# GuidoManni/BodySLAM

Measured on AMD Instinct MI355X. Metric: frames/sec depth+pose+back-proj, 640x480 seq, higher is better.
Workload: dtype f16

## Files before the change

bodyslam_amd/csrc/igemm_kernel.h:

```cpp
#pragma once
#include <type_traits>

#include "common.h"

namespace bs {

struct IgemmParams {
    const void* A;
    const void* W;
    const void* zero;
    long long a_bytes;
    int M, N, K, lda;
    int Hin, Win, Cin, Hout, Wout, KH, KW, stride, pad_h, pad_w;
    int tiles_per_tap;
    int cin1;
    int split_off;
    int res_split_off;
    int relu_a;
    const float* bias;
    int bias_group_rows;
    int act;
    const float* scale;
    const void* res;
    const void* res2;
    int res_dtype, ldr;
    void* out;
    void* out2;
    void* out3;
    int out_dtype, ldo, out_mode;
    int out_group_rows, out_group_stride, out_row_offset;
    int shuffle_s, shuffle_cout;
    int qkv_hidden, qkv_tokens, qkv_sp;
    int qkv_cls_last;
    int qkv_cls_rows;
    int qkv_patch_row0;
    int qkv_lo_off;
    int f8_wonly_from;
    float q_scale;
    int ntm, ntn;
    int m_begin;
    int f8_seg;
    int f8_sa0, f8_sb0, f8_sa1, f8_sb1;
    int f8_stages;
    int res_f8;
    int out_f8;
    int out2_relu;
    int out_lo8_rows;
    int f8_skip_from;
    int out_planes_rows;
    const float* bias2;
    int bias2_row0, bias2_group_rows;
    int strip;
    int ablate;
};

template <typename T>
__device__ __forceinline__ typename T16<T>::v8 relu8(typename T16<T>::v8 x) {
    typedef short s16x8 __attribute__((ext_vector_type(8)));
    s16x8 b = __builtin_bit_cast(s16x8, x);
    s16x8 neg = b >> 15;
    b = b & ~neg;
    return __builtin_bit_cast(typename T16<T>::v8, b);
}

template <typename T>
__device__ __forceinline__ void store4(void* base, int64_t off, int out_dtype, const float (&y)[4], int split_off = 0) {
    if (split_off > 0) {
        typename T16<T>::v4 h, l;
#pragma unroll
        for (int e = 0; e < 4; ++e) {
            h[e] = T16<T>::from_f32(y[e]);
            l[e] = T16<T>::from_f32(y[e] - T16<T>::to_f32(h[e]));
        }
        *reinterpret_cast<typename T16<T>::v4*>(reinterpret_cast<T*>(base) + off) = h;
        *reinterpret_cast<typename T16<T>::v4*>(reinterpret_cast<T*>(base) + off + split_off) = l;
        return;
    }
    if (out_dtype == BS_F32) {
        f32x4 v = {y[0], y[1], y[2], y[3]};
        *reinterpret_cast<f32x4*>(reinterpret_cast<float*>(base) + off) = v;
    } else {
        typename T16<T>::v4 v;
        v[0] = T16<T>::from_f32(y[0]);
        v[1] = T16<T>::from_f32(y[1]);
        v[2] = T16<T>::from_f32(y[2]);
        v[3] = T16<T>::from_f32(y[3]);
        *reinterpret_cast<typename T16<T>::v4*>(reinterpret_cast<T*>(base) + off) = v;
    }
}

template <typename T>
__device__ __forceinline__ void store8(void* base, int64_t off, int out_dtype, const float (&y)[8], int split_off = 0) {
    typedef typename T16<T>::v8 v8;
    if (split_off > 0) {
        v8 h, l;
#pragma unroll
        for (int e = 0; e < 8; ++e) {
            h[e] = T16<T>::from_f32(y[e]);
            l[e] = T16<T>::from_f32(y[e] - T16<T>::to_f32(h[e]));
        }
        *reinterpret_cast<v8*>(reinterpret_cast<T*>(base) + off) = h;
        *reinterpret_cast<v8*>(reinterpret_cast<T*>(base) + off + split_off) = l;
        return;
    }
    if (out_dtype == BS_F32) {
        *reinterpret_cast<f32x4*>(reinterpret_cast<float*>(base) + off) = f32x4{y[0], y[1], y[2], y[3]};
        *reinterpret_cast<f32x4*>(reinterpret_cast<float*>(base) + off + 4) = f32x4{y[4], y[5], y[6], y[7]};
    } else {
        v8 v;
#pragma unroll
        for (int e = 0; e < 8; ++e) v[e] = T16<T>::from_f32(y[e]);
        *reinterpret_cast<v8*>(reinterpret_cast<T*>(base) + off) = v;
    }
}

template <typename T>
__device__ __forceinline__ void store8_f8(void* base, int64_t row_off, int n, int plane_off, const float (&y)[8], int ea, int el, bool lo = true,
                                          bool hi8 = true) {
    typedef typename T16<T>::v8 v8;
    typedef int i32x2 __attribute__((ext_vector_type(2)));
    v8 h;
    f32x2_ yh[4];
    const float sa = __builtin_ldexpf(1.0f, ea), sl = __builtin_ldexpf(1.0f, el);
    const f32x2_ sa2 = {sa, sa}, sl2 = {sl, sl};
#pragma unroll
    for (int e = 0; e < 8; e += 2) {
        h[e] = T16<T>::from_f32(y[e]);
        h[e + 1] = T16<T>::from_f32(y[e + 1]);
        const f32x2_ v = f32x2_{y[e], y[e + 1]} * sa2;
        yh[e >> 1] = f32x2_{__builtin_amdgcn_fmed3f(v[0], -448.0f, 448.0f), __builtin_amdgcn_fmed3f(v[1], -448.0f, 448.0f)};
    }
    T* rowp = reinterpret_cast<T*>(base) + row_off;
    *reinterpret_cast<v8*>(rowp + n) = h;
    if (!hi8) return;
    int ph0 = 0, ph1 = 0;
    ph0 = __builtin_amdgcn_cvt_pk_fp8_f32(yh[0][0], yh[0][1], ph0, false);
    ph0 = __builtin_amdgcn_cvt_pk_fp8_f32(yh[1][0], yh[1][1], ph0, true);
    ph1 = __builtin_amdgcn_cvt_pk_fp8_f32(yh[2][0], yh[2][1], ph1, false);
    ph1 = __builtin_amdgcn_cvt_pk_fp8_f32(yh[3][0], yh[3][1], ph1, true);
    char* bytes = reinterpret_cast<char*>(rowp + plane_off);
    *reinterpret_cast<i32x2*>(bytes + n) = i32x2{ph0, ph1};
    if (lo) {
        f32x2_ yl[4];
#pragma unroll
        for (int e = 0; e < 8; e += 2) {
            const f32x2_ r = (f32x2_{y[e], y[e + 1]} + f32x2_{-T16<T>::to_f32(h[e]), -T16<T>::to_f32(h[e + 1])}) * sl2;
            yl[e >> 1] = f32x2_{__builtin_amdgcn_fmed3f(r[0], -448.0f, 448.0f), __builtin_amdgcn_fmed3f(r[1], -448.0f, 448.0f)};
        }
        int pl0 = 0, pl1 = 0;
        pl0 = __builtin_amdgcn_cvt_pk_fp8_f32(yl[0][0], yl[0][1], pl0, false);
        pl0 = __builtin_amdgcn_cvt_pk_fp8_f32(yl[1][0], yl[1][1], pl0, true);
        pl1 = __builtin_amdgcn_cvt_pk_fp8_f32(yl[2][0], yl[2][1], pl1, false);
        pl1 = __builtin_amdgcn_cvt_pk_fp8_f32(yl[3][0], yl[3][1], pl1, true);
        *reinterpret_cast<i32x2*>(bytes + plane_off + n) = i32x2{pl0, pl1};
    }
}

template <typename T>
__device__ __forceinline__ void add_lo8(float* y, const void* base, int64_t row_off, int C, int n) {
    const char* lp = reinterpret_cast<const char*>(reinterpret_cast<const T*>(base) + row_off + C + (C >> 1)) + n;
    const int packed = *reinterpret_cast<const int*>(lp);
    typedef float f32x2 __attribute__((ext_vector_type(2)));
    const f32x2 a = __builtin_amdgcn_cvt_pk_f32_fp8(packed, false), b = __builtin_amdgcn_cvt_pk_f32_fp8(packed, true);
    const float sc = __builtin_ldexpf(1.0f, -BS_F8_ACT_LO_EXP);
    y[0] += a[0] * sc; y[1] += a[1] * sc; y[2] += b[0] * sc; y[3] += b[1] * sc;
}

constexpr int NW_CHECK(int a, int b) { return a * b; }

template <int N>
__device__ __forceinline__ void wait_vmcnt() {
    asm volatile("s_waitcnt vmcnt(%0)" ::"n"(N) : "memory");
}

template <typename T, int BM, int BN, int WM, int WN, int BK, int STAGES, int MODE, bool PP = false, int CM = 0, int SCHED = 0>
__global__ __launch_bounds__(WM* WN * 64, 2) void igemm_kernel(const IgemmParams p) {
#if defined(__HIP_DEVICE_COMPILE__)
    constexpr bool CONV = MODE != 0;
    constexpr bool RELU_A = MODE == 2;
    constexpr bool F8 = CM != 0;
    constexpr int NT = WM * WN * 64;
    constexpr int ROWB = BK * 2;
    constexpr int LPR = ROWB / 16;
    constexpr int RPR = NT / LPR;
    constexpr int RPW = 64 / LPR;
    constexpr int RA = BM / RPR, RB = BN / RPR;
    static_assert(BK == 64 || BK == 32, "BK");
    static_assert(BM % RPR == 0 && BN % RPR == 0, "tile rows must be a multiple of the DMA round");
    constexpr int GL = RA + RB;
    static_assert(GL * (STAGES - 1) <= 63, "vmcnt range");
    constexpr int TM = BM / WM, TN = BN / WN;
    constexpr int FM = TM / 16, FN = TN / 16;
    static_assert(TM % 16 == 0 && TN % 16 == 0, "wave tile must be a multiple of 16");
    constexpr int A_BYTES = BM * ROWB, B_BYTES = BN * ROWB, STAGE = A_BYTES + B_BYTES;
    constexpr int LDS_BYTES = STAGES * STAGE;
    constexpr unsigned OOB = 0x80000000u;
    typedef typename T16<T>::v8 v8;

    extern __shared__ __attribute__((aligned(16))) char smem[];

    const int nwg = gridDim.x, bid = blockIdx.x;
    const int xq = nwg >> 3, xr = nwg & 7, xcd = bid & 7, loc = bid >> 3;
    const int wg = (xcd < xr ? xcd * (xq + 1) : xr * (xq + 1) + (xcd - xr) * xq) + loc;
    int tm, tn;
    if (p.strip > 0) {
        const int per = p.ntm * p.strip, s = wg / per, r = wg - s * per;
        const int wl = p.ntn - s * p.strip < p.strip ? p.ntn - s * p.strip : p.strip;
        tm = r / wl;
        tn = s * p.strip + (r - tm * wl);
    } else {
        tm = wg / p.ntn;
        tn = wg - tm * p.ntn;
    }

    const int tid = threadIdx.x, lane = tid & 63;
    const int wave = __builtin_amdgcn_readfirstlane(tid >> 6);
    const int wm = wave / WN, wn = wave - wm * WN;
    const int srow = tid / LPR;
    const int sswz = (BK == 64) ? (srow & 7) : ((0 - (srow >> 2)) & 3);
    const int cs16 = ((tid & (LPR - 1)) ^ sswz) * 16;

    const int m0 = p.m_begin + tm * BM;
    long long a_base_el;
    int img0 = 0;
    if (CONV) {
        img0 = m0 / (p.Hout * p.Wout);
        a_base_el = (long long)img0 * p.Hin * p.Win * p.lda;
    } else {
        a_base_el = (long long)m0 * p.lda;
    }
    long long a_left = p.a_bytes - a_base_el * 2;
    a_left = a_left > 0x7FFFFFF0ll ? 0x7FFFFFF0ll : a_left;
    const __amdgpu_buffer_rsrc_t a_rsrc = __builtin_amdgcn_make_buffer_rsrc(
        const_cast<T*>(reinterpret_cast<const T*>(p.A)) + a_base_el, 0, (int)a_left, 0x00020000);
    const int w_pitch = p.K * 2;
    const __amdgpu_buffer_rsrc_t w_rsrc = __builtin_amdgcn_make_buffer_rsrc(
        const_cast<void*>(p.W), 0, (int)((long long)p.N * w_pitch), 0x00020000);

    unsigned a_off[RA];
    unsigned a_mask[RA];
#pragma unroll
    for (int j = 0; j < RA; ++j) {
        int m = m0 + j * RPR + srow;
        m = m < p.M ? m : p.M - 1;
        if (CONV) {
            const int hw = p.Hout * p.Wout;
            const int b = m / hw, rem = m - b * hw;
            const int oy = rem / p.Wout, ox = rem - oy * p.Wout;
            const int iy0 = oy * p.stride - p.pad_h, ix0 = ox * p.stride - p.pad_w;
            a_off[j] = (unsigned)((((b - img0) * p.Hin + iy0) * p.Win + ix0) * p.lda * 2 + cs16);
            unsigned mk = 0;
            for (int ky = 0; ky < p.KH; ++ky)
                for (int kx = 0; kx < p.KW; ++kx) {
                    const bool ok = (unsigned)(iy0 + ky) < (unsigned)p.Hin && (unsigned)(ix0 + kx) < (unsigned)p.Win;
                    mk |= (ok ? 1u : 0u) << (ky * p.KW + kx);
                }
            a_mask[j] = mk;
        } else {
            a_off[j] = (unsigned)((m - m0) * p.lda * 2 + cs16);
            a_mask[j] = 1u;
        }
    }
    static_assert(BN % 32 == 0 && TN % 32 == 0, "column permutation works on 32-column groups");
    unsigned w_off[RB];
#pragma unroll
    for (int j = 0; j < RB; ++j) {
        int r = j * RPR + srow;
        if (SCHED == 1) r = (((r >> 5) & 3) << 6) | ((r >> 7) << 5) | (r & 31);
        int n = tn * BN + ((r & ~31) | ((r & 12) << 1) | ((r & 16) >> 2) | (r & 3));
        n = n < p.N ? n : p.N - 1;
        w_off[j] = (unsigned)(n * w_pitch + cs16);
    }
    const int seg0 = (CONV ? p.Cin : p.K - p.cin1) * 2, seg1 = p.cin1 * 2;
    const int ntaps = CONV ? p.KH * p.KW : 1;
    int s_tap = 0, s_kx = 0, s_tapoff = 0, s_cb = 0, s_sub = 0, s_k = 0, s_seg = seg0;

    auto stage_advance = [&]() {
        s_k += BK * 2;
        if (BK == 32) {
            s_sub ^= 64;
            if (s_sub) return;
        }
        if (CONV) {
            ++s_tap;
            s_tapoff += p.lda * 2;
            if (++s_kx >= p.KW) {
                s_kx = 0;
                s_tapoff += (p.Win - p.KW) * p.lda * 2;
            }
        }
        if (!CONV || s_tap >= ntaps) {
            s_tap = 0;
            s_kx = 0;
            s_tapoff = 0;
            s_cb += 128;
            if (s_cb >= s_seg) {
                s_cb = 0;
                s_seg = seg1;
            }
        }
    };
    auto stage = [&](int buf) {
        char* sa = smem + buf * STAGE;
        char* sb = sa + A_BYTES;
        const int s_c0 = s_cb + s_sub;
#pragma unroll
        for (int j = 0; j < RA; ++j) {
            unsigned vo;
// ... 425 lines not shown
                }
                float yall[FN / 2][8];
#pragma unroll
                for (int jp = 0; jp < FN / 2; ++jp) {
                    float (&y8)[8] = yall[jp];
#pragma unroll
                    for (int h = 0; h < 2; ++h) {
                        const int j = jp * 2 + h;
                        float* y = y8 + h * 4;
                        if (n0j[j] >= p.N) continue;
                        f32x4 bsum = brow ? *reinterpret_cast<const f32x4*>(brow + n0j[j]) : bj[j];
                        if (brow2) bsum += *reinterpret_cast<const f32x4*>(brow2 + n0j[j]);
#pragma unroll
                        for (int e = 0; e < 4; ++e) y[e] = acc[i][j][e] + bsum[e];
                        const bool res32 = p.res && p.res_dtype == BS_F32;
                        if (ACT == BS_ACT_GELU) {
                            const f32x2_ g0 = gelu_erf2(f32x2_{y[0], y[1]}), g1 = gelu_erf2(f32x2_{y[2], y[3]});
                            y[0] = g0[0]; y[1] = g0[1]; y[2] = g1[0]; y[3] = g1[1];
                        }
#pragma unroll
                        for (int e = 0; e < 4; ++e) {
                            if (ACT == BS_ACT_RELU) y[e] = fmaxf(y[e], 0.0f);
                            else if (ACT == BS_ACT_SOFTPLUS) y[e] = softplus20(y[e]);
                            else if (ACT == BS_ACT_SOFTPLUS_FAST) y[e] = softplus_fast(y[e]);
                            if (!res32) y[e] *= sj[j][e];
                        }
                        if (p.res) {
                            const int64_t ro = orow * p.ldr + n0j[j];
                            if (p.res_dtype == BS_F32) {
                                const f32x4 rr = *reinterpret_cast<const f32x4*>(reinterpret_cast<const float*>(p.res) + ro);
#pragma unroll
                                for (int e = 0; e < 4; ++e) y[e] = __builtin_fmaf(y[e], sj[j][e], rr[e]);
                            } else {
                                const typename T16<T>::v4 rr = *reinterpret_cast<const typename T16<T>::v4*>(reinterpret_cast<const T*>(p.res) + ro);
#pragma unroll
                                for (int e = 0; e < 4; ++e) y[e] += T16<T>::to_f32(rr[e]);
                                if (p.res_split_off > 0) {
                                    const typename T16<T>::v4 rl = *reinterpret_cast<const typename T16<T>::v4*>(reinterpret_cast<const T*>(p.res) + ro + p.res_split_off);
#pragma unroll
                                    for (int e = 0; e < 4; ++e) y[e] += T16<T>::to_f32(rl[e]);
                                } else if (F8 && p.res_f8) {
                                    add_lo8<T>(y, p.res, orow * p.ldr, p.N, n0j[j]);
                                }
                            }
                            if (p.res2) {
                                const typename T16<T>::v4 rr = *reinterpret_cast<const typename T16<T>::v4*>(reinterpret_cast<const T*>(p.res2) + ro);
#pragma unroll
                                for (int e = 0; e < 4; ++e) y[e] += T16<T>::to_f32(rr[e]);
                                if (p.res_split_off > 0) {
                                    const typename T16<T>::v4 rl = *reinterpret_cast<const typename T16<T>::v4*>(reinterpret_cast<const T*>(p.res2) + ro + p.res_split_off);
#pragma unroll
                                    for (int e = 0; e < 4; ++e) y[e] += T16<T>::to_f32(rl[e]);
                                } else if (F8 && p.res_f8) {
                                    add_lo8<T>(y, p.res2, orow * p.ldr, p.N, n0j[j]);
                                }
                            }
                        }
                    }
                }
#pragma unroll
                for (int jp = 0; jp < FN / 2; ++jp) {
                    float (&y8)[8] = yall[jp];
                    const int j0 = jp * 2, j1 = j0 + 1;
                    if (n0j[j0] >= p.N) continue;
                    void* dst = (p.out_mode == BS_OUT_QKV && which[j0] == 1) ? p.out2 : p.out;
                    const int so = p.out_mode != BS_OUT_QKV ? p.split_off : p.qkv_lo_off;
                    if (F8 && p.out_f8) {
                        const int nloc = p.out_mode == BS_OUT_SHUFFLE ? n0j[j0] % p.shuffle_cout : n0j[j0];
                        store8_f8<T>(dst, roff + coff[j0] - nloc, nloc, so, y8, p.out_f8 & 0xff, (p.out_f8 >> 8) & 0xff);
                    } else if (wide_ok && n0j[j1] < p.N && coff[j1] == coff[j0] + 4 && which[j1] == which[j0]) {
                        store8<T>(dst, roff + coff[j0], p.out_dtype, y8, so);
                    } else {
                        const float(&ya)[4] = *reinterpret_cast<const float(*)[4]>(y8);
                        store4<T>(dst, roff + coff[j0], p.out_dtype, ya, so);
                        if (n0j[j1] < p.N) {
                            const float(&yb)[4] = *reinterpret_cast<const float(*)[4]>(y8 + 4);
                            void* dst1 = (p.out_mode == BS_OUT_QKV && which[j1] == 1) ? p.out2 : p.out;
                            store4<T>(dst1, roff + coff[j1], p.out_dtype, yb, so);
                        }
                    }
                }
            }
        };
        const bool plain_full = p.out_mode == BS_OUT_PLAIN && !p.out_group_rows && p.bias && !p.bias_group_rows && p.N % BN == 0 &&
                                p.ldo % 8 == 0 && !b2_rows && !(p.ablate & 16);
        if (plain_full && p.act == BS_ACT_NONE && p.res && p.res_dtype == BS_F32 && !p.res2 && p.out_dtype == BS_F32 && p.split_off == 0 &&
            !(F8 && p.out_f8) && p.scale && p.ldr % 4 == 0) {
            BS_FRESH_LANE
            constexpr int NP = FM * (FN / 2), DEPTH = 8;
            const float* resp = reinterpret_cast<const float*>(p.res);
            float* outp = reinterpret_cast<float*>(p.out);
            f32x4 bj[FN], sj[FN];
#pragma unroll
            for (int j = 0; j < FN; ++j) {
                const int n0 = n_wave + (j >> 1) * 32 + fq * 8 + (j & 1) * 4;
                bj[j] = *reinterpret_cast<const f32x4*>(p.bias + n0);
                if (g2 >= 0) bj[j] += *reinterpret_cast<const f32x4*>(p.bias2 + (int64_t)g2 * p.N + n0);
                sj[j] = *reinterpret_cast<const f32x4*>(p.scale + n0);
            }
            const int mrow = m0 + wm * TM + frow;
            f32x4 rq[DEPTH][2];
            auto issue = [&](int it, int slot) {
                const int i = it / (FN / 2), jp = it - i * (FN / 2);
                int m = mrow + i * 16;
                m = m < p.M ? m : p.M - 1;
                const float* rp = resp + (int64_t)m * p.ldr + n_wave + jp * 32 + fq * 8;
                rq[slot][0] = *reinterpret_cast<const f32x4*>(rp);
                rq[slot][1] = *reinterpret_cast<const f32x4*>(rp + 4);
            };
#pragma unroll
            for (int it = 0; it < DEPTH; ++it) issue(it, it);
#pragma unroll
            for (int it = 0; it < NP; ++it) {
                const int i = it / (FN / 2), jp = it - i * (FN / 2);
                const int m = mrow + i * 16;
                f32x4 y0, y1;
#pragma unroll
                for (int e = 0; e < 4; ++e) {
                    y0[e] = __builtin_fmaf(acc[i][2 * jp][e] + bj[2 * jp][e], sj[2 * jp][e], rq[it % DEPTH][0][e]);
                    y1[e] = __builtin_fmaf(acc[i][2 * jp + 1][e] + bj[2 * jp + 1][e], sj[2 * jp + 1][e], rq[it % DEPTH][1][e]);
                }
                if (it + DEPTH < NP) issue(it + DEPTH, it % DEPTH);
                if (m < p.M) {
                    float* op = outp + (int64_t)m * p.ldo + n_wave + jp * 32 + fq * 8;
                    *reinterpret_cast<f32x4*>(op) = y0;
                    *reinterpret_cast<f32x4*>(op + 4) = y1;
                }
            }
            return;
        }
        if constexpr (F8) {
            if (p.out_mode == BS_OUT_PLAIN && !p.out_group_rows && !p.bias_group_rows && p.N % BN == 0 && p.ldo % 8 == 0 && !b2_rows &&
                !(p.ablate & (16 | 2048)) && p.out_f8 && !p.scale && (p.act == BS_ACT_NONE || p.act == BS_ACT_RELU) && p.split_off == p.N &&
                p.N % 8 == 0 && p.out_dtype != BS_F32 &&
                (!p.res || (p.res_f8 && p.res_dtype != BS_F32 && p.res_split_off == 0 && p.ldr % 8 == 0)) && (!p.res2 || p.res)) {
                BS_FRESH_LANE
                typedef typename T16<T>::v8 v8;
                typedef int i32x2 __attribute__((ext_vector_type(2)));
                typedef float f32x2 __attribute__((ext_vector_type(2)));
                constexpr int NP = FM * (FN / 2), RDEPTH = 4;
                f32x4 bj[FN];
#pragma unroll
                for (int j = 0; j < FN; ++j) {
                    const int n0 = n_wave + (j >> 1) * 32 + fq * 8 + (j & 1) * 4;
                    bj[j] = p.bias ? *reinterpret_cast<const f32x4*>(p.bias + n0) : f32x4{0.f, 0.f, 0.f, 0.f};
                    if (g2 >= 0) bj[j] += *reinterpret_cast<const f32x4*>(p.bias2 + (int64_t)g2 * p.N + n0);
                }
                const bool relu = p.act == BS_ACT_RELU;
                const int mrow = m0 + wm * TM + frow;
                const int ea = p.out_f8 & 0xff, el = (p.out_f8 >> 8) & 0xff;
                const bool lo_plane = !(p.out_lo8_rows > 0 && m0 >= p.out_lo8_rows);
                const bool hi_plane = !(p.out_planes_rows > 0 && m0 >= p.out_planes_rows);
                const float lsc = __builtin_ldexpf(1.0f, -BS_F8_ACT_LO_EXP);
                auto body = [&](auto nres_tag) {
                    constexpr int NRES = decltype(nres_tag)::value;
                    v8 rh[NRES ? RDEPTH : 1][NRES ? NRES : 1];
                    i32x2 rl[NRES ? RDEPTH : 1][NRES ? NRES : 1];
                    auto issue = [&](int it, int slot) {
                        const int i = it / (FN / 2), jp = it - i * (FN / 2);
                        int m = mrow + i * 16;
                        m = m < p.M ? m : p.M - 1;
                        const int n = n_wave + jp * 32 + fq * 8;
#pragma unroll
                        for (int q = 0; q < NRES; ++q) {
                            const T* rp = reinterpret_cast<const T*>(q ? p.res2 : p.res) + (int64_t)m * p.ldr;
                            rh[slot][q] = *reinterpret_cast<const v8*>(rp + n);
                            rl[slot][q] = *reinterpret_cast<const i32x2*>(reinterpret_cast<const char*>(rp + p.N + (p.N >> 1)) + n);
                        }
                    };
                    if constexpr (NRES > 0) {
#pragma unroll
                        for (int it = 0; it < RDEPTH; ++it) issue(it, it);
                    }
#pragma unroll
                    for (int it = 0; it < NP; ++it) {
                        const int i = it / (FN / 2), jp = it - i * (FN / 2);
                        const int m = mrow + i * 16;
                        float y8[8];
#pragma unroll
                        for (int h = 0; h < 2; ++h)
#pragma unroll
                            for (int e = 0; e < 4; ++e) {
                                float y = acc[i][2 * jp + h][e] + bj[2 * jp + h][e];
                                if (relu) y = fmaxf(y, 0.0f);
                                y8[4 * h + e] = y;
                            }
                        if constexpr (NRES > 0) {
#pragma unroll
                            for (int q = 0; q < NRES; ++q) {
                                const v8 hv = rh[it % RDEPTH][q];
                                const i32x2 lv = rl[it % RDEPTH][q];
#pragma unroll
                                for (int h = 0; h < 2; ++h) {
#pragma unroll
                                    for (int e = 0; e < 4; ++e) y8[4 * h + e] += T16<T>::to_f32(hv[4 * h + e]);
                                    const f32x2 a = __builtin_amdgcn_cvt_pk_f32_fp8(lv[h], false), b = __builtin_amdgcn_cvt_pk_f32_fp8(lv[h], true);
                                    y8[4 * h] += a[0] * lsc; y8[4 * h + 1] += a[1] * lsc; y8[4 * h + 2] += b[0] * lsc; y8[4 * h + 3] += b[1] * lsc;
                                }
                            }
                            if (it + RDEPTH < NP) issue(it + RDEPTH, it % RDEPTH);
                        }
                        if (m < p.M) store8_f8<T>(p.out, (int64_t)m * p.ldo, n_wave + jp * 32 + fq * 8, p.split_off, y8, ea, el, lo_plane && hi_plane, hi_plane);
                        if (p.out2_relu) {
#pragma unroll
                            for (int e = 0; e < 8; ++e) y8[e] = fmaxf(y8[e], 0.0f);
                            if (m < p.M) store8_f8<T>(p.out2, (int64_t)m * p.ldo, n_wave + jp * 32 + fq * 8, p.split_off, y8, ea, el);
                        }
                    }
                };
                if (p.res2) body(std::integral_constant<int, 2>{});
                else if (p.res) body(std::integral_constant<int, 1>{});
                else body(std::integral_constant<int, 0>{});
                return;
            }
            if (plain_full && p.act == BS_ACT_GELU && !p.res && p.out_f8 && !p.scale && p.split_off == p.N && p.N % 8 == 0) {
                BS_FRESH_LANE
                const bool lo = !(p.out_lo8_rows > 0 && m0 >= p.out_lo8_rows);
                const bool planes = !(p.out_planes_rows > 0 && m0 >= p.out_planes_rows);
                f32x4 bj[FN];
#pragma unroll
                for (int j = 0; j < FN; ++j) {
                    const int n0 = n_wave + (j >> 1) * 32 + fq * 8 + (j & 1) * 4;
                    bj[j] = *reinterpret_cast<const f32x4*>(p.bias + n0);
                    if (g2 >= 0) bj[j] += *reinterpret_cast<const f32x4*>(p.bias2 + (int64_t)g2 * p.N + n0);
                }
                if constexpr (TM == 128 && TN == 64 && LDS_BYTES >= WM * WN * 16384) {
                    if (!planes && m0 + BM <= p.M && !(p.ablate & 1024)) {
                        typedef unsigned u32x4_ __attribute__((ext_vector_type(4)));
                        __syncthreads();
                        char* sw = smem + wave * 16384;
                        const int s7 = frow & 7;
                        const int wb0 = frow * 128 + ((fq ^ s7) << 4), wb1 = frow * 128 + (((4 + fq) ^ s7) << 4);
                        const int rr = lane >> 3, pc = lane & 7;
                        const int rb = rr * 128 + ((pc ^ rr) << 4);
                        T* op = reinterpret_cast<T*>(p.out) + (int64_t)(m0 + wm * TM + rr) * p.ldo + n_wave + pc * 8;
                        const int64_t step = (int64_t)8 * p.ldo;
#pragma unroll
                        for (int ip = 0; ip < FM; ip += 2) {
                            char* sr = sw + ((ip >> 1) & 1) * 4096;
#pragma unroll
                            for (int ii = 0; ii < 2; ++ii) {
                                const int i = ip + ii;
#pragma unroll
                                for (int jp = 0; jp < FN / 2; ++jp) {
                                    typename T16<T>::v8 h8v;
#pragma unroll
                                    for (int h = 0; h < 2; ++h) {
                                        const f32x4 v = acc[i][2 * jp + h] + bj[2 * jp + h];
                                        const f32x2_ g0 = gelu_erf2(f32x2_{v[0], v[1]}), g1 = gelu_erf2(f32x2_{v[2], v[3]});
                                        h8v[4 * h] = T16<T>::from_f32(g0[0]); h8v[4 * h + 1] = T16<T>::from_f32(g0[1]);
                                        h8v[4 * h + 2] = T16<T>::from_f32(g1[0]); h8v[4 * h + 3] = T16<T>::from_f32(g1[1]);
                                    }
                                    *reinterpret_cast<typename T16<T>::v8*>(sr + (jp ? wb1 : wb0) + ii * 2048) = h8v;
                                }
                            }
                            __builtin_amdgcn_fence(__ATOMIC_RELEASE, "wavefront");
                            __builtin_amdgcn_wave_barrier();
#pragma unroll
                            for (int it = 0; it < 4; ++it) {
                                *reinterpret_cast<u32x4_*>(op) = *reinterpret_cast<const u32x4_*>(sr + rb + it * 1024);
                                op += step;
                            }
                        }
                        return;
                    }
                }
#pragma unroll
                for (int i = 0; i < FM; ++i) {
                    const int m = m0 + wm * TM + i * 16 + frow;
                    if (m >= p.M) continue;
#pragma unroll
                    for (int jp = 0; jp < FN / 2; ++jp) {
                        float y8[8];
#pragma unroll
                        for (int h = 0; h < 2; ++h) {
                            const f32x4 v = acc[i][2 * jp + h] + bj[2 * jp + h];
                            const f32x2_ g0 = gelu_erf2(f32x2_{v[0], v[1]}), g1 = gelu_erf2(f32x2_{v[2], v[3]});
                            y8[4 * h] = g0[0]; y8[4 * h + 1] = g0[1]; y8[4 * h + 2] = g1[0]; y8[4 * h + 3] = g1[1];
                        }
                        if (planes) {
                            store8_f8<T>(p.out, (int64_t)m * p.ldo, n_wave + jp * 32 + fq * 8, p.split_off, y8, p.out_f8 & 0xff, (p.out_f8 >> 8) & 0xff, lo);
                        } else {
                            typename T16<T>::v8 h;
#pragma unroll
                            for (int e = 0; e < 8; ++e) h[e] = T16<T>::from_f32(y8[e]);
                            *reinterpret_cast<typename T16<T>::v8*>(reinterpret_cast<T*>(p.out) + (int64_t)m * p.ldo + n_wave + jp * 32 + fq * 8) = h;
                        }
                    }
                }
                return;
            }
        }
        if (F8 && p.out_mode == BS_OUT_QKV && p.qkv_hidden % BN == 0 && p.act == BS_ACT_NONE && !p.res && p.bias && !p.bias_group_rows && !b2_rows &&
            p.out_dtype != BS_F32 && !(p.ablate & 16)) {
            BS_FRESH_LANE
            const int part = (tn * BN) / p.qkv_hidden;
            T* dst = reinterpret_cast<T*>(part == 1 ? p.out2 : p.out);
            const float qs = part == 0 ? p.q_scale : 1.0f;
            f32x4 bj[FN], sj[FN];
            int64_t coff[FN / 2];
#pragma unroll
            for (int j = 0; j < FN; ++j) {
                const int n0 = n_wave + (j >> 1) * 32 + fq * 8 + (j & 1) * 4;
                bj[j] = *reinterpret_cast<const f32x4*>(p.bias + n0);
                if (g2 >= 0) bj[j] += *reinterpret_cast<const f32x4*>(p.bias2 + (int64_t)g2 * p.N + n0);
                sj[j] = p.scale ? *reinterpret_cast<const f32x4*>(p.scale + n0) : f32x4{1.f, 1.f, 1.f, 1.f};
#pragma unroll
                for (int e = 0; e < 4; ++e) sj[j][e] *= qs;
                if (!(j & 1)) {
                    const int rem = n0 - part * p.qkv_hidden;
                    coff[j >> 1] = (int64_t)(rem >> 6) * p.qkv_sp * 64 + (rem & 63);
                }
            }
            const int nhead = p.qkv_hidden >> 6;
            const long long q_bytes = (long long)p.qkv_cls_rows * nhead * p.qkv_sp * 128;
            if (p.qkv_cls_rows > 0 && m0 >= p.qkv_patch_row0 && p.qkv_lo_off == 0 && !(p.ablate & (128 | 256)) && q_bytes < 0x7FFFFFF0ll) {
                typedef unsigned u32x4_ __attribute__((ext_vector_type(4)));
                const __amdgpu_buffer_rsrc_t orsrc = __builtin_amdgcn_make_buffer_rsrc(dst, 0, (int)q_bytes, 0x00020000);
                const int Tk = p.qkv_tokens - 1;
                int m = m0 + wm * TM + frow;
                const int mp0 = m - p.qkv_patch_row0;
                const int ob0 = mp0 / Tk;
                int otok = mp0 - ob0 * Tk;
                const unsigned img_bytes = (unsigned)(nhead * p.qkv_sp) * 128u;
                unsigned roff = (unsigned)ob0 * img_bytes + (unsigned)otok * 128u;
                if constexpr (TM == 128 && TN == 64 && LDS_BYTES >= WM * WN * 16384) {
                    if (m0 + BM <= p.M && Tk % 8 == 0 && (m0 - p.qkv_patch_row0) % 8 == 0 && !(p.ablate & 1024)) {
                        __syncthreads();
                        char* sw = smem + wave * 16384;
                        const int s7 = frow & 7;
                        const int wb0 = frow * 128 + ((fq ^ s7) << 4), wb1 = frow * 128 + (((4 + fq) ^ s7) << 4);
#pragma unroll
                        for (int i = 0; i < FM; ++i) {
#pragma unroll
                            for (int jp = 0; jp < FN / 2; ++jp) {
                                typename T16<T>::v8 v;
#pragma unroll
                                for (int e = 0; e < 4; ++e) {
                                    v[e] = T16<T>::from_f32((acc[i][2 * jp][e] + bj[2 * jp][e]) * sj[2 * jp][e]);
                                    v[4 + e] = T16<T>::from_f32((acc[i][2 * jp + 1][e] + bj[2 * jp + 1][e]) * sj[2 * jp + 1][e]);
                                }
                                *reinterpret_cast<typename T16<T>::v8*>(sw + (jp ? wb1 : wb0) + i * 2048) = v;
                            }
                        }
                        __builtin_amdgcn_fence(__ATOMIC_RELEASE, "wavefront");
                        __builtin_amdgcn_wave_barrier();
                        const int rr = lane >> 3, pc = lane & 7;
                        const int mpl = m0 + wm * TM + rr - p.qkv_patch_row0;
                        const int obl = mpl / Tk;
                        int tokl = mpl - obl * Tk;
                        const int rem0 = n_wave - part * p.qkv_hidden;
                        unsigned ro = (unsigned)obl * img_bytes + (unsigned)tokl * 128u + (unsigned)(rem0 >> 6) * (unsigned)p.qkv_sp * 128u + pc * 16u;
                        const int rb = rr * 128 + ((pc ^ rr) << 4);
#pragma unroll
                        for (int it = 0; it < 16; ++it) {
                            const u32x4_ x = *reinterpret_cast<const u32x4_*>(sw + rb + it * 1024);
                            __builtin_amdgcn_raw_buffer_store_b128(x, orsrc, ro, 0, 0);
                            tokl += 8;
                            ro += 8u * 128u;
                            if (tokl >= Tk) {
                                tokl -= Tk;
                                ro += img_bytes - (unsigned)Tk * 128u;
                            }
                        }
                        return;
                    }
// ... 231 lines not shown
```

Baseline: 489.9.

## Stage fp8 split-plane epilogue stores through LDS for coalesced row writes

Splits store8_f8 into a conversion helper and a store, then adds an LDS-staged epilogue for the 64x64 wave tile. Per-lane scattered 16-byte and 8-byte writes of the f16 high plane and the fp8 hi/lo planes are first written to swizzled shared memory, then flushed as full contiguous row segments. The same staging is applied to the residual epilogue and to a new pixel-shuffle output path. The aim is better global store coalescing, at the cost of extra LDS traffic, wave barriers and more shared-memory use per wave.

```diff
diff --git a/bodyslam_amd/csrc/igemm_kernel.h b/bodyslam_amd/csrc/igemm_kernel.h
--- a/bodyslam_amd/csrc/igemm_kernel.h
+++ b/bodyslam_amd/csrc/igemm_kernel.h
@@ -114,12 +114,9 @@
     }
 }
 
+typedef int i32x2_ __attribute__((ext_vector_type(2)));
 template <typename T>
-__device__ __forceinline__ void store8_f8(void* base, int64_t row_off, int n, int plane_off, const float (&y)[8], int ea, int el, bool lo = true,
-                                          bool hi8 = true) {
-    typedef typename T16<T>::v8 v8;
-    typedef int i32x2 __attribute__((ext_vector_type(2)));
-    v8 h;
+__device__ __forceinline__ void cvt8_f8(const float (&y)[8], int ea, int el, bool lo, bool hi8, typename T16<T>::v8& h, i32x2_& ph, i32x2_& pl) {
     f32x2_ yh[4];
     const float sa = __builtin_ldexpf(1.0f, ea), sl = __builtin_ldexpf(1.0f, el);
     const f32x2_ sa2 = {sa, sa}, sl2 = {sl, sl};
@@ -130,16 +127,13 @@
         const f32x2_ v = f32x2_{y[e], y[e + 1]} * sa2;
         yh[e >> 1] = f32x2_{__builtin_amdgcn_fmed3f(v[0], -448.0f, 448.0f), __builtin_amdgcn_fmed3f(v[1], -448.0f, 448.0f)};
     }
-    T* rowp = reinterpret_cast<T*>(base) + row_off;
-    *reinterpret_cast<v8*>(rowp + n) = h;
     if (!hi8) return;
     int ph0 = 0, ph1 = 0;
     ph0 = __builtin_amdgcn_cvt_pk_fp8_f32(yh[0][0], yh[0][1], ph0, false);
     ph0 = __builtin_amdgcn_cvt_pk_fp8_f32(yh[1][0], yh[1][1], ph0, true);
     ph1 = __builtin_amdgcn_cvt_pk_fp8_f32(yh[2][0], yh[2][1], ph1, false);
     ph1 = __builtin_amdgcn_cvt_pk_fp8_f32(yh[3][0], yh[3][1], ph1, true);
-    char* bytes = reinterpret_cast<char*>(rowp + plane_off);
-    *reinterpret_cast<i32x2*>(bytes + n) = i32x2{ph0, ph1};
+    ph = i32x2_{ph0, ph1};
     if (lo) {
         f32x2_ yl[4];
 #pragma unroll
@@ -152,8 +146,75 @@
         pl0 = __builtin_amdgcn_cvt_pk_fp8_f32(yl[1][0], yl[1][1], pl0, true);
         pl1 = __builtin_amdgcn_cvt_pk_fp8_f32(yl[2][0], yl[2][1], pl1, false);
         pl1 = __builtin_amdgcn_cvt_pk_fp8_f32(yl[3][0], yl[3][1], pl1, true);
-        *reinterpret_cast<i32x2*>(bytes + plane_off + n) = i32x2{pl0, pl1};
-    }
+        pl = i32x2_{pl0, pl1};
+    }
+}
+
+template <typename T>
+__device__ __forceinline__ void store8_f8(void* base, int64_t row_off, int n, int plane_off, const float (&y)[8], int ea, int el, bool lo = true,
+                                          bool hi8 = true) {
+    typename T16<T>::v8 h;
+    i32x2_ ph = {0, 0}, pl = {0, 0};
+    cvt8_f8<T>(y, ea, el, lo, hi8, h, ph, pl);
+    T* rowp = reinterpret_cast<T*>(base) + row_off;
+    *reinterpret_cast<typename T16<T>::v8*>(rowp + n) = h;
+    if (!hi8) return;
+    char* bytes = reinterpret_cast<char*>(rowp + plane_off);
+    *reinterpret_cast<i32x2_*>(bytes + n) = ph;
+    if (lo) *reinterpret_cast<i32x2_*>(bytes + plane_off + n) = pl;
+}
+
+struct StageOffsets {
+    int wb[2], pb[2], rb, qb;
+};
+__device__ __forceinline__ StageOffsets stage_offsets(int lane) {
+    const int frow = lane & 15, fq = lane >> 4, rr = lane >> 3, pc = lane & 7;
+    StageOffsets o;
+#pragma unroll
+    for (int jp = 0; jp < 2; ++jp) {
+        o.wb[jp] = frow * 128 + (((jp * 4 + fq) ^ (frow & 7)) << 4);
+        o.pb[jp] = frow * 64 + (((jp * 4 + fq) ^ (frow >> 1)) << 3);
+    }
+    o.rb = rr * 128 + ((pc ^ rr) << 4);
+    o.qb = rr * 64 + ((pc ^ (rr >> 1)) << 3);
+    return o;
+}
+template <typename T>
+__device__ __forceinline__ void stage8_f8(char* sr, const StageOffsets& o, int ii, int jp, const typename T16<T>::v8& h, const i32x2_& ph, const i32x2_& pl,
+                                          bool lo, bool hi8) {
+    *reinterpret_cast<typename T16<T>::v8*>(sr + o.wb[jp] + ii * 2048) = h;
+    if (!hi8) return;
+    *reinterpret_cast<i32x2_*>(sr + 4096 + o.pb[jp] + ii * 1024) = ph;
+    if (lo) *reinterpret_cast<i32x2_*>(sr + 6144 + o.pb[jp] + ii * 1024) = pl;
+}
+template <typename T>
+__device__ __forceinline__ void flush_rows32(const char* sr, const StageOffsets& o, T* const (&rowp)[4], int col, int plane_off, bool lo, bool hi8) {
+    typedef unsigned u32x4_ __attribute__((ext_vector_type(4)));
+    __builtin_amdgcn_fence(__ATOMIC_RELEASE, "wavefront");
+    __builtin_amdgcn_wave_barrier();
+#pragma unroll
+    for (int k = 0; k < 4; ++k) {
+        const u32x4_ x = *reinterpret_cast<const u32x4_*>(sr + o.rb + k * 1024);
+        if (rowp[k]) *reinterpret_cast<u32x4_*>(rowp[k] + col) = x;
+    }
+    __builtin_amdgcn_sched_barrier(0);
+    if (hi8) {
+#pragma unroll
+        for (int k = 0; k < 4; ++k) {
+            const i32x2_ x = *reinterpret_cast<const i32x2_*>(sr + 4096 + (o.qb ^ ((k & 1) << 5)) + k * 512);
+            if (rowp[k]) *reinterpret_cast<i32x2_*>(reinterpret_cast<char*>(rowp[k] + plane_off) + col) = x;
+        }
+        __builtin_amdgcn_sched_barrier(0);
+        if (lo) {
+#pragma unroll
+            for (int k = 0; k < 4; ++k) {
+                const i32x2_ x = *reinterpret_cast<const i32x2_*>(sr + 6144 + (o.qb ^ ((k & 1) << 5)) + k * 512);
+                if (rowp[k]) *reinterpret_cast<i32x2_*>(reinterpret_cast<char*>(rowp[k] + plane_off) + plane_off + col) = x;
+            }
+        }
+    }
+    __builtin_amdgcn_fence(__ATOMIC_RELEASE, "wavefront");
+    __builtin_amdgcn_wave_barrier();
 }
 
 template <typename T>
@@ -885,8 +946,13 @@
                 const bool lo_plane = !(p.out_lo8_rows > 0 && m0 >= p.out_lo8_rows);
                 const bool hi_plane = !(p.out_planes_rows > 0 && m0 >= p.out_planes_rows);
                 const float lsc = __builtin_ldexpf(1.0f, -BS_F8_ACT_LO_EXP);
+                constexpr bool CAN_STAGE = TM == 64 && TN == 64 && LDS_BYTES >= WM * WN * 16384;
+                const bool staged = CAN_STAGE && !(p.ablate & 64);
                 auto body = [&](auto nres_tag) {
                     constexpr int NRES = decltype(nres_tag)::value;
+                    const StageOffsets so = stage_offsets(lane);
+                    char* sw = smem + wave * 16384;
+                    if (staged) __syncthreads();
                     v8 rh[NRES ? RDEPTH : 1][NRES ? NRES : 1];
                     i32x2 rl[NRES ? RDEPTH : 1][NRES ? NRES : 1];
                     auto issue = [&](int it, int slot) {
@@ -933,11 +999,43 @@
                             }
                             if (it + RDEPTH < NP) issue(it + RDEPTH, it % RDEPTH);
                         }
-                        if (m < p.M) store8_f8<T>(p.out, (int64_t)m * p.ldo, n_wave + jp * 32 + fq * 8, p.split_off, y8, ea, el, lo_plane && hi_plane, hi_plane);
-                        if (p.out2_relu) {
-#pragma unroll
-                            for (int e = 0; e < 8; ++e) y8[e] = fmaxf(y8[e], 0.0f);
-                            if (m < p.M) store8_f8<T>(p.out2, (int64_t)m * p.ldo, n_wave + jp * 32 + fq * 8, p.split_off, y8, ea, el);
+                        if constexpr (CAN_STAGE) if (staged) {
+                            const int grp = i >> 1;
+                            char* sr = sw + (p.out2_relu ? 0 : (grp & 1) * 8192);
+                            v8 h;
+                            i32x2_ ph = {0, 0}, pl = {0, 0};
+                            cvt8_f8<T>(y8, ea, el, lo_plane && hi_plane, hi_plane, h, ph, pl);
+                            stage8_f8<T>(sr, so, i & 1, jp, h, ph, pl, lo_plane && hi_plane, hi_plane);
+                            if (p.out2_relu) {
+#pragma unroll
+                                for (int e = 0; e < 8; ++e) y8[e] = fmaxf(y8[e], 0.0f);
+                                cvt8_f8<T>(y8, ea, el, true, true, h, ph, pl);
+                                stage8_f8<T>(sr + 8192, so, i & 1, jp, h, ph, pl, true, true);
+                            }
+                            if ((i & 1) && jp == FN / 2 - 1) {
+                                const int mr = m0 + wm * TM + grp * 32 + (lane >> 3);
+                                const int col = n_wave + (lane & 7) * 8;
+                                T* rowp[4];
+#pragma unroll
+                                for (int k = 0; k < 4; ++k)
+                                    rowp[k] = mr + k * 8 < p.M ? reinterpret_cast<T*>(p.out) + (int64_t)(mr + k * 8) * p.ldo : nullptr;
+                                flush_rows32<T>(sr, so, rowp, col, p.split_off, lo_plane && hi_plane, hi_plane);
+                                if (p.out2_relu) {
+#pragma unroll
+                                    for (int k = 0; k < 4; ++k)
+                                        rowp[k] = mr + k * 8 < p.M ? reinterpret_cast<T*>(p.out2) + (int64_t)(mr + k * 8) * p.ldo : nullptr;
+                                    flush_rows32<T>(sr + 8192, so, rowp, col, p.split_off, true, true);
+                                }
+                            }
+                            continue;
+                        }
+                        {
+                            if (m < p.M) store8_f8<T>(p.out, (int64_t)m * p.ldo, n_wave + jp * 32 + fq * 8, p.split_off, y8, ea, el, lo_plane && hi_plane, hi_plane);
+                            if (p.out2_relu) {
+#pragma unroll
+                                for (int e = 0; e < 8; ++e) y8[e] = fmaxf(y8[e], 0.0f);
+                                if (m < p.M) store8_f8<T>(p.out2, (int64_t)m * p.ldo, n_wave + jp * 32 + fq * 8, p.split_off, y8, ea, el);
+                            }
                         }
                     }
                 };
@@ -945,6 +1043,69 @@
                 else if (p.res) body(std::integral_constant<int, 1>{});
                 else body(std::integral_constant<int, 0>{});
                 return;
+            }
+            if constexpr (TM == 64 && TN == 64 && LDS_BYTES >= WM * WN * 16384) {
+                if (p.out_mode == BS_OUT_SHUFFLE && p.out_f8 && !p.scale && !p.res && !p.bias_group_rows && !p.bias2 && p.N % BN == 0 &&
+                    p.shuffle_cout % 64 == 0 && p.ldo % 8 == 0 && p.split_off % 16 == 0 && p.Wout >= 8 &&
+                    (p.act == BS_ACT_NONE || p.act == BS_ACT_RELU) && p.out_dtype != BS_F32 && !(p.ablate & (16 | 64))) {
+                    BS_FRESH_LANE
+                    f32x4 bj[FN];
+#pragma unroll
+                    for (int j = 0; j < FN; ++j) {
+                        const int n0 = n_wave + (j >> 1) * 32 + fq * 8 + (j & 1) * 4;
+                        bj[j] = p.bias ? *reinterpret_cast<const f32x4*>(p.bias + n0) : f32x4{0.f, 0.f, 0.f, 0.f};
+                    }
+                    const bool relu = p.act == BS_ACT_RELU;
+                    const int ea = p.out_f8 & 0xff, el = (p.out_f8 >> 8) & 0xff;
+                    const int s = p.shuffle_s, tap = n_wave / p.shuffle_cout, co0 = n_wave - tap * p.shuffle_cout;
+                    const int ky = tap / s, kx = tap - ky * s;
+                    T* outp = reinterpret_cast<T*>(p.out) + ((int64_t)ky * (p.Wout * s) + kx) * p.ldo;
+                    int mr = m0 + wm * TM + (lane >> 3);
+                    const int R = mr / p.Wout;
+                    int ox = mr - R * p.Wout;
+                    int64_t pix = (int64_t)R * s * (p.Wout * s) + ox * s;
+                    const int wrap = p.Wout * s * (s - 1);
+                    const int col = co0 + (lane & 7) * 8;
+                    __syncthreads();
+                    const StageOffsets so = stage_offsets(lane);
+                    char* sw = smem + wave * 16384;
+#pragma unroll
+                    for (int i = 0; i < FM; ++i) {
+                        char* sr = sw + ((i >> 1) & 1) * 8192;
+#pragma unroll
+                        for (int jp = 0; jp < FN / 2; ++jp) {
+                            float y8[8];
+#pragma unroll
+                            for (int h = 0; h < 2; ++h)
+#pragma unroll
+                                for (int e = 0; e < 4; ++e) {
+                                    float y = acc[i][2 * jp + h][e] + bj[2 * jp + h][e];
+                                    if (relu) y = fmaxf(y, 0.0f);
+                                    y8[4 * h + e] = y;
+                                }
+                            typename T16<T>::v8 h;
+                            i32x2_ ph = {0, 0}, pl = {0, 0};
+                            cvt8_f8<T>(y8, ea, el, true, true, h, ph, pl);
+                            stage8_f8<T>(sr, so, i & 1, jp, h, ph, pl, true, true);
+                        }
+                        if (i & 1) {
+                            T* rowp[4];
+#pragma unroll
+                            for (int k = 0; k < 4; ++k) {
+                                rowp[k] = mr < p.M ? outp + pix * p.ldo : nullptr;
+                                mr += 8;
+                                ox += 8;
+                                pix += 8 * s;
+                                if (ox >= p.Wout) {
+                                    ox -= p.Wout;
+                                    pix += wrap;
+                                }
+                            }
+                            flush_rows32<T>(sr, so, rowp, col, p.split_off, true, true);
+                        }
+                    }
+                    return;
+                }
             }
             if (plain_full && p.act == BS_ACT_GELU && !p.res && p.out_f8 && !p.scale && p.split_off == p.N && p.N % 8 == 0) {
                 BS_FRESH_LANE
```

Measured after the change: 489.7. Within noise of the previous version (-0.0%).
